# gmlwns2000/sharkshark-4k

Hardware: AMD Instinct MI355X
Metric: upscaled frames/sec at 720p->1440p x2 (whole job) (higher is better)
Workload: dtype f16; 1 GPU; RealESRGAN RRDBNet x2 (23 blocks) 720p->1440p fp16 [BASELINE configs[2]]; io=uint8 NHWC resident in HBM

## Files before the change

### include/ss4k_dev.h

```cpp
#ifndef SS4K_DEV_H
#define SS4K_DEV_H
#include "ss4k.h"
#ifdef __cplusplus
extern "C" {
#endif


int ss4k_bench_conv(ss4k_ctx* ctx, int dtype, int cin0, int cin1, int cout, int n, int h, int w, int flags,
                    int iters, double* avg_us, void* hip_stream);

int ss4k_dev_op_area_normalized(ss4k_ctx* ctx, const void* in, int in_half, float* out, int planes, int h, int w, int oh,
                                int ow, const float* st_hr, const float* st_lr, void* hip_stream);
int ss4k_dev_op_tail_fused(ss4k_ctx* ctx, void* hr, int hr_half, uint8_t* out_u8, const float* diff, int n, int c, int h,
                           int w, int dh, int dw, const float* st_hr, const float* st_lr, void* hip_stream);
int ss4k_dev_op_bicubic_u8(ss4k_ctx* ctx, const void* in, int in_half, uint8_t* out, int n, int c, int h, int w, int oh,
                           int ow, void* hip_stream);
int ss4k_dev_op_bicubic(ss4k_ctx* ctx, const float* in, float* out, int planes, int h, int w, int oh, int ow, int clamp01,
                        void* hip_stream);
int ss4k_dev_op_bilinear(ss4k_ctx* ctx, const float* in, float* out, int planes, int h, int w, int oh, int ow,
                         int subtract_from_out, int clamp01, void* hip_stream);
int ss4k_dev_gauss17_taps(float* taps17);
int ss4k_dev_op_gauss17_reflect(ss4k_ctx* ctx, const float* in, float* tmp, float* out, const float* taps17_dev, int planes,
                                int h, int w, void* hip_stream);
int ss4k_dev_op_depthwise_reflect(ss4k_ctx* ctx, const float* in, float* out, const float* taps_dev, int planes, int h,
                                  int w, int k, int clamp01, const float* blend_src, float blend_a, float blend_b,
                                  void* hip_stream);
int ss4k_dev_op_normalize(ss4k_ctx* ctx, float* x, const float* st_hr, const float* st_lr, int planes, int hw, void* hip_stream);
int ss4k_dev_op_sub(ss4k_ctx* ctx, const float* a, const float* b, float* out, size_t n, void* hip_stream);
int ss4k_dev_op_clamp01(ss4k_ctx* ctx, float* x, size_t n, void* hip_stream);
int ss4k_dev_op_plane_stats(ss4k_ctx* ctx, double* acc, const void* in, int in_half, float* stats, int planes, int hw,
                            void* hip_stream);
int ss4k_dev_op_plane_stats_u8nhwc(ss4k_ctx* ctx, double* acc, const uint8_t* in, float* stats, int n, int hw, void* hip_stream);
int ss4k_dev_op_plane_stats_partial(ss4k_ctx* ctx, double* acc, const void* in, int in_half, int planes, int hw,
                                    int acc_planes, int plane0, void* hip_stream);
int ss4k_dev_op_plane_stats_u8nhwc_partial(ss4k_ctx* ctx, double* acc, const uint8_t* in, int n, int hw, int acc_planes,
                                           int plane0, void* hip_stream);
int ss4k_dev_op_plane_stats_finish(ss4k_ctx* ctx, const double* acc, float* stats, int planes, int hw, void* hip_stream);
int ss4k_dev_op_plane_stats_finish2(ss4k_ctx* ctx, double* acc, float* stats_a, float* stats_b, int planes, int hw_a,
                                    int hw_b, int rezero, void* hip_stream);
int ss4k_dev_op_ps_nchw_addbase(ss4k_ctx* ctx, const void* src, int src_half, void* out, int out_half, const float* base,
                                int n, int h, int w, int r, int cq, double* stats_acc, void* hip_stream);
int ss4k_dev_op_pack_input(ss4k_ctx* ctx, const float* in, void* out, int out_half, int n, int c, int h, int w, int r,
                           int nplanes, void* hip_stream);
int ss4k_dev_op_temporal_shift(ss4k_ctx* ctx, const void* in, void* out, int nplanes, int frames, size_t frame_px,
                               int slots_per_record, int ch_per_plane, int fold, void* hip_stream);

int ss4k_dev_op_frvsr_maxpool2_planes(ss4k_ctx* ctx, const void* in, void* out, int half, int nplanes, int n, int h, int w, void* hip_stream);
int ss4k_dev_op_frvsr_bilinear2_planes(ss4k_ctx* ctx, const void* in, void* out, int half, int nplanes, int n, int h, int w, void* hip_stream);
int ss4k_dev_op_frvsr_flow_finish(ss4k_ctx* ctx, const float* raw, float* flow, int n, int h8, int w8, int h, int w, void* hip_stream);
int ss4k_dev_op_frvsr_warp_s2d_planes(ss4k_ctx* ctx, const float* lr_flow, const float* hr_prev, void* out, int half, int n, int h, int w,
                                      void* hip_stream);
int ss4k_dev_op_frvsr_warp_s2d_planes_items(ss4k_ctx* ctx, const float* lr_flow, const float* const* hr_prev, void* out, int half, int n,
                                            int h, int w, void* hip_stream);
int ss4k_dev_op_frvsr_ps4_conv_tail(ss4k_ctx* ctx, const void* in, int half, const float* wb, float* out, int n, int h, int w, void* hip_stream);
int ss4k_dev_op_frvsr_ps4_conv_tail_items(ss4k_ctx* ctx, const void* in, int half, const float* wb, float* const* out, int n, int h, int w,
                                          void* hip_stream);
int ss4k_dev_op_frvsr_planes_to_nchw(ss4k_ctx* ctx, const void* in, int half, float* out, int n, int channels, int h, int w, void* hip_stream);
int ss4k_dev_op_frvsr_clamp01_to(ss4k_ctx* ctx, const float* in, float* out, size_t n, void* hip_stream);
int ss4k_dev_op_frvsr_frames_in_items(ss4k_ctx* ctx, const uint8_t* const* in, float* const* lr_curr, int n, int h, int w, int lh, int lw,
                                      void* hip_stream);
int ss4k_dev_op_frvsr_pack_lr_items(ss4k_ctx* ctx, const float* const* lr_curr, const float* const* lr_prev, void* a, void* b, int half, int n,
                                    int h, int w, void* hip_stream);
int ss4k_dev_op_frvsr_frames_out_items(ss4k_ctx* ctx, const float* const* hr, uint8_t* const* out, int n, int H, int W, int oh, int ow,
                                       void* hip_stream);

int ss4k_dev_op_frvsrbi_bilinear_upsample4(ss4k_ctx* ctx, const float* in, float* out, int planes, int h, int w, void* hip_stream);
int ss4k_dev_op_frvsrbi_warp_s2d_planes(ss4k_ctx* ctx, const float* lr_flow, const float* hr_prev, void* out, int half, int n, int h, int w,
                                         void* hip_stream);
int ss4k_dev_op_frvsrbi_warp_s2d_planes_items(ss4k_ctx* ctx, const float* lr_flow, const float* const* hr_prev, void* out, int half, int n,
                                               int h, int w, void* hip_stream);
int ss4k_dev_op_frvsrbi_bilinear4_add(ss4k_ctx* ctx, const float* conv, const float* lr, float* out, int n, int h, int w, void* hip_stream);
int ss4k_dev_op_frvsrbi_bilinear4_add_items(ss4k_ctx* ctx, const float* conv, const float* const* lr, float* const* out, int n, int h, int w,
                                          void* hip_stream);

int ss4k_dev_frvsr_step_taps(ss4k_frvsr* m, const float* lr_curr, const float* lr_prev, const float* hr_prev, float* hr_out, float* flow_out,
                             float* s2d_out, int n, int h, int w, void* hip_stream);

int ss4k_dev_frvsr_tail_taps(ss4k_frvsr* m, const float* body_nchw, const float* lr_curr, float* up1_out, float* up2_out, float* hr_out, int n, int h,
                             int w, int max_workgroups, int group_items, void* hip_stream);
int ss4k_dev_frvsr_embed_convt(const float* wt_and_bias, int nf, float* out, size_t capacity_floats);
int ss4k_dev_frvsr_pack_convt(const float* wt, int dtype, void* out, size_t capacity_bytes);

int ss4k_dev_op_spin(ss4k_ctx* ctx, unsigned ticks, void* hip_stream);
int ss4k_dev_lane_handicap(ss4k_ctx* ctx, int lane, unsigned ticks);
int ss4k_dev_lane_counts(ss4k_ctx* ctx, int64_t* forks, int64_t* joins, int64_t* spins);
int ss4k_dev_lane_counts_reset(ss4k_ctx* ctx);
int ss4k_dev_lane_drop_join(ss4k_ctx* ctx, int k);

int ss4k_dev_glue_routes_reset(void);
int ss4k_dev_glue_routes_read(int index, char* name, size_t name_capacity, int64_t* launches);

int ss4k_dev_guard_enable(int on);
int ss4k_dev_guard_check(int* guarded, int* unguarded, int* damaged, char* text, size_t text_capacity);
int ss4k_dev_guard_poison(ss4k_ctx* ctx, ss4k_model* model, ss4k_upscaler* upscaler, int* buffers, size_t* bytes, size_t* bytes_256);
int ss4k_dev_guard_poison_frvsr(ss4k_frvsr* m, ss4k_frvsr_upscaler* up, int* buffers, size_t* bytes, size_t* bytes_256);
int ss4k_dev_guard_selftest(ss4k_ctx* ctx);

#ifdef __cplusplus
}
#endif
#endif
```

### sharkshark-4k_amd/_capi.py

```python
from __future__ import annotations

import ctypes as C
import os
from typing import Optional, Sequence, Tuple

import numpy as np
import torch

_HERE = os.path.dirname(os.path.abspath(__file__))
LIB_PATH = os.environ.get("SS4K_LIB") or os.path.join(_HERE, "libss4k_hip.so")

FSRCNN, RRDBNET, SRVGG, BSVD = 1, 2, 3, 4
F32, F16 = 0, 1

SYMBOLS = [
    "ss4k_abi_version", "ss4k_last_error", "ss4k_ctx_create", "ss4k_ctx_destroy", "ss4k_ctx_device",
    "ss4k_model_param_count", "ss4k_model_create", "ss4k_model_destroy", "ss4k_model_out_shape",
    "ss4k_model_in_channels", "ss4k_model_forward", "ss4k_model_check", "ss4k_upscaler_create", "ss4k_upscaler_destroy",
    "ss4k_upscaler_reset", "ss4k_upscaler_out_shape", "ss4k_upscaler_last_enqueue_ms", "ss4k_model_workspace_bytes", "ss4k_upscale_frames", "ss4k_upscaler_enable_taps",
    "ss4k_upscaler_read_tap", "ss4k_op_u8nhwc_to_f32nchw", "ss4k_op_area_resize", "ss4k_op_bicubic_resize",
    "ss4k_op_bilinear_resize", "ss4k_op_depthwise_reflect", "ss4k_op_plane_stats", "ss4k_op_f32nchw_to_u8nhwc",
    "ss4k_prof_enable", "ss4k_prof_reset", "ss4k_prof_read", "ss4k_prof_read_kind", "ss4k_prof_read_family", "ss4k_prof_read_section_ms",
    "ss4k_stream_pair_check", "ss4k_op_cv_area_shape", "ss4k_op_cv_area_resize_u8",
    "ss4k_frvsr_param_count", "ss4k_frvsr_create", "ss4k_frvsr_destroy", "ss4k_frvsr_step", "ss4k_frvsr_workspace_bytes",
    "ss4k_frvsr_prof_enable", "ss4k_frvsr_prof_read", "ss4k_frvsr_upscaler_create", "ss4k_frvsr_upscaler_destroy",
    "ss4k_frvsr_upscaler_reset", "ss4k_frvsr_upscaler_out_shape", "ss4k_frvsr_upscale_frames", "ss4k_frvsr_upscaler_enable_taps",
    "ss4k_frvsr_upscaler_read_tap", "ss4k_op_backward_warp", "ss4k_op_bicubic_upsample4",
    "ss4k_frvsr_upscaler_create_streams", "ss4k_frvsr_upscale_streams", "ss4k_frvsr_upscaler_reset_stream", "ss4k_frvsr_upscaler_state_bytes",
    "ss4k_frvsr_upscale_streams_at",
    "ss4k_frvsr_param_count_as", "ss4k_frvsr_create_as", "ss4k_frvsr_generator",
    "ss4k_frvsr_param_count_ex", "ss4k_frvsr_create_ex", "ss4k_frvsr_degradation",
]
DEV_SYMBOLS = [
    "ss4k_bench_conv",
    "ss4k_dev_op_area_normalized", "ss4k_dev_op_tail_fused", "ss4k_dev_op_bicubic_u8", "ss4k_dev_op_bicubic", "ss4k_dev_op_bilinear",
    "ss4k_dev_gauss17_taps", "ss4k_dev_op_gauss17_reflect", "ss4k_dev_op_depthwise_reflect", "ss4k_dev_op_normalize", "ss4k_dev_op_sub",
    "ss4k_dev_op_clamp01", "ss4k_dev_op_plane_stats", "ss4k_dev_op_plane_stats_u8nhwc", "ss4k_dev_op_plane_stats_partial",
    "ss4k_dev_op_plane_stats_u8nhwc_partial", "ss4k_dev_op_plane_stats_finish", "ss4k_dev_op_plane_stats_finish2",
    "ss4k_dev_op_ps_nchw_addbase", "ss4k_dev_op_pack_input", "ss4k_dev_op_temporal_shift",
    "ss4k_dev_glue_routes_reset", "ss4k_dev_glue_routes_read",
    "ss4k_dev_op_frvsr_maxpool2_planes", "ss4k_dev_op_frvsr_bilinear2_planes", "ss4k_dev_op_frvsr_flow_finish",
    "ss4k_dev_op_frvsr_warp_s2d_planes", "ss4k_dev_op_frvsr_warp_s2d_planes_items", "ss4k_dev_op_frvsr_ps4_conv_tail",
    "ss4k_dev_op_frvsr_ps4_conv_tail_items", "ss4k_dev_op_frvsr_planes_to_nchw", "ss4k_dev_op_frvsr_clamp01_to",
    "ss4k_dev_op_frvsr_frames_in_items", "ss4k_dev_op_frvsr_pack_lr_items", "ss4k_dev_op_frvsr_frames_out_items",
    "ss4k_dev_op_frvsrbi_bilinear_upsample4", "ss4k_dev_op_frvsrbi_warp_s2d_planes", "ss4k_dev_op_frvsrbi_warp_s2d_planes_items",
    "ss4k_dev_op_frvsrbi_bilinear4_add", "ss4k_dev_op_frvsrbi_bilinear4_add_items",
    "ss4k_dev_frvsr_step_taps",
    "ss4k_dev_frvsr_tail_taps", "ss4k_dev_frvsr_embed_convt", "ss4k_dev_frvsr_pack_convt",
    "ss4k_dev_guard_enable", "ss4k_dev_guard_check", "ss4k_dev_guard_poison", "ss4k_dev_guard_selftest", "ss4k_dev_guard_poison_frvsr",
    "ss4k_dev_op_spin", "ss4k_dev_lane_handicap", "ss4k_dev_lane_counts", "ss4k_dev_lane_counts_reset", "ss4k_dev_lane_drop_join",
]


class ModelDesc(C.Structure):
    _fields_ = [("kind", C.c_int32), ("dtype", C.c_int32), ("scale", C.c_int32), ("num_feat", C.c_int32),
                ("num_block", C.c_int32), ("num_grow_ch", C.c_int32), ("bsvd_chns", C.c_int32 * 3),
                ("bsvd_mid_ch", C.c_int32), ("bsvd_interm_ch", C.c_int32), ("bsvd_stream", C.c_int32),
                ("flags", C.c_int32), ("reserved", C.c_int32 * 3)]


MODEL_FS_EXACT, MODEL_ONE_CHAIN, MODEL_TWO_CHAINS, MODEL_TILE_ROWS_16, MODEL_TILE_ROWS_20 = 1, 2, 4, 16, 32
MODEL_NO_PAIR, MODEL_HR_F32, MODEL_NO_DENSE, MODEL_NO_WIDE, MODEL_NO_UPS_PRESUM, MODEL_NO_W16 = 256, 512, 1024, 4096, 8192, 32768
MODEL_FLAGS_ALL = 1 | 2 | 4 | 16 | 32 | 256 | 512 | 1024 | 4096 | 8192 | 32768


class UpscaleCfg(C.Structure):
    _fields_ = [("lr_h", C.c_int32), ("lr_w", C.c_int32), ("out_h", C.c_int32), ("out_w", C.c_int32),
                ("lr_hr_resize", C.c_int32), ("single_mode", C.c_int32), ("sr_is_realesrgan", C.c_int32),
                ("denoising", C.c_int32), ("reserved0", C.c_int32), ("denoise_rate", C.c_double),
                ("reserved", C.c_int32 * 6)]


class FrvsrDesc(C.Structure):
    _fields_ = [("dtype", C.c_int32), ("num_feat", C.c_int32), ("num_block", C.c_int32), ("flags", C.c_int32),
                ("reserved", C.c_int32 * 4)]


class Ss4kError(RuntimeError):
    pass


_lib = None
GPU_TOUCHED = False


def lib() -> C.CDLL:
    global _lib
    if _lib is None:
        _lib = load(LIB_PATH)
    return _lib


def load(path: str) -> C.CDLL:
    if not os.path.exists(path):
        raise Ss4kError(f"{path} is missing: build it with `python -c 'import __graft_entry__ as g; g.build()'`")
    L = C.CDLL(path)
    vp, i, sz = C.c_void_p, C.c_int, C.c_size_t
    L.ss4k_last_error.restype = C.c_char_p
    L.ss4k_ctx_create.argtypes = [i, C.POINTER(vp)]
    L.ss4k_ctx_destroy.argtypes = [vp]; L.ss4k_ctx_destroy.restype = None
    L.ss4k_ctx_device.argtypes = [vp]
    L.ss4k_model_param_count.argtypes = [C.POINTER(ModelDesc)]; L.ss4k_model_param_count.restype = sz
    L.ss4k_model_create.argtypes = [vp, C.POINTER(ModelDesc), vp, sz, C.POINTER(vp)]
    L.ss4k_model_destroy.argtypes = [vp]; L.ss4k_model_destroy.restype = None
    L.ss4k_model_out_shape.argtypes = [vp, i, i, i, C.POINTER(i), C.POINTER(i), C.POINTER(i)]
    L.ss4k_model_in_channels.argtypes = [vp]
    L.ss4k_model_forward.argtypes = [vp, vp, vp, i, i, i, vp]
    if hasattr(L, "ss4k_model_check"):
        L.ss4k_model_check.argtypes = [vp, i]
    L.ss4k_upscaler_create.argtypes = [vp, C.POINTER(UpscaleCfg), vp, vp, C.POINTER(vp)]
    L.ss4k_upscaler_destroy.argtypes = [vp]; L.ss4k_upscaler_destroy.restype = None
    L.ss4k_upscaler_reset.argtypes = [vp]
    L.ss4k_model_workspace_bytes.argtypes = [vp, i, i, i, C.POINTER(C.c_size_t)]
    L.ss4k_upscaler_last_enqueue_ms.argtypes = [vp, C.POINTER(C.c_double), C.POINTER(C.c_double)]
    L.ss4k_upscaler_out_shape.argtypes = [vp, i, i, i, C.POINTER(i), C.POINTER(i)]
    L.ss4k_upscale_frames.argtypes = [vp, vp, i, i, i, vp, sz, vp]
    L.ss4k_upscaler_enable_taps.argtypes = [vp, i]
    L.ss4k_upscaler_read_tap.argtypes = [vp, i, vp, sz, C.POINTER(i * 4), vp]
    L.ss4k_op_u8nhwc_to_f32nchw.argtypes = [vp, vp, vp, i, i, i, i, vp]
    for name in ("ss4k_op_area_resize", "ss4k_op_bicubic_resize", "ss4k_op_bilinear_resize"):
        getattr(L, name).argtypes = [vp, vp, vp, i, i, i, i, i, vp]
    L.ss4k_op_depthwise_reflect.argtypes = [vp, vp, vp, i, i, i, vp, i, vp]
    L.ss4k_op_plane_stats.argtypes = [vp, vp, vp, i, i, vp]
    L.ss4k_op_f32nchw_to_u8nhwc.argtypes = [vp, vp, vp, i, i, i, i, vp]
    if hasattr(L, "ss4k_bench_conv"):
        L.ss4k_bench_conv.argtypes = [vp, i, i, i, i, i, i, i, i, i, C.POINTER(C.c_double), vp]
    if hasattr(L, "ss4k_dev_glue_routes_read"):
        f = C.c_float
        L.ss4k_dev_op_area_normalized.argtypes = [vp, vp, i, vp, i, i, i, i, i, vp, vp, vp]
        L.ss4k_dev_op_tail_fused.argtypes = [vp, vp, i, vp, vp, i, i, i, i, i, i, vp, vp, vp]
        L.ss4k_dev_op_bicubic_u8.argtypes = [vp, vp, i, vp, i, i, i, i, i, i, vp]
        L.ss4k_dev_op_bicubic.argtypes = [vp, vp, vp, i, i, i, i, i, i, vp]
        L.ss4k_dev_op_bilinear.argtypes = [vp, vp, vp, i, i, i, i, i, i, i, vp]
        L.ss4k_dev_gauss17_taps.argtypes = [vp]
        L.ss4k_dev_op_gauss17_reflect.argtypes = [vp, vp, vp, vp, vp, i, i, i, vp]
        L.ss4k_dev_op_depthwise_reflect.argtypes = [vp, vp, vp, vp, i, i, i, i, i, vp, f, f, vp]
        L.ss4k_dev_op_normalize.argtypes = [vp, vp, vp, vp, i, i, vp]
        L.ss4k_dev_op_sub.argtypes = [vp, vp, vp, vp, sz, vp]
        L.ss4k_dev_op_clamp01.argtypes = [vp, vp, sz, vp]
        L.ss4k_dev_op_plane_stats.argtypes = [vp, vp, vp, i, vp, i, i, vp]
        L.ss4k_dev_op_plane_stats_u8nhwc.argtypes = [vp, vp, vp, vp, i, i, vp]
        L.ss4k_dev_op_plane_stats_partial.argtypes = [vp, vp, vp, i, i, i, i, i, vp]
        L.ss4k_dev_op_plane_stats_u8nhwc_partial.argtypes = [vp, vp, vp, i, i, i, i, vp]
        L.ss4k_dev_op_plane_stats_finish.argtypes = [vp, vp, vp, i, i, vp]
        L.ss4k_dev_op_plane_stats_finish2.argtypes = [vp, vp, vp, vp, i, i, i, i, vp]
        L.ss4k_dev_op_ps_nchw_addbase.argtypes = [vp, vp, i, vp, i, vp, i, i, i, i, i, vp, vp]
        L.ss4k_dev_op_pack_input.argtypes = [vp, vp, vp, i, i, i, i, i, i, i, vp]
        L.ss4k_dev_op_temporal_shift.argtypes = [vp, vp, vp, i, i, sz, i, i, i, vp]
        L.ss4k_dev_glue_routes_reset.argtypes = []
        L.ss4k_dev_op_frvsr_maxpool2_planes.argtypes = [vp, vp, vp, i, i, i, i, i, vp]
        L.ss4k_dev_op_frvsr_bilinear2_planes.argtypes = [vp, vp, vp, i, i, i, i, i, vp]
        L.ss4k_dev_op_frvsr_flow_finish.argtypes = [vp, vp, vp, i, i, i, i, i, vp]
        L.ss4k_dev_op_frvsr_warp_s2d_planes.argtypes = [vp, vp, vp, vp, i, i, i, i, vp]
        L.ss4k_dev_op_frvsr_warp_s2d_planes_items.argtypes = [vp, vp, vp, vp, i, i, i, i, vp]
        L.ss4k_dev_op_frvsr_ps4_conv_tail.argtypes = [vp, vp, i, vp, vp, i, i, i, vp]
        L.ss4k_dev_op_frvsr_ps4_conv_tail_items.argtypes = [vp, vp, i, vp, vp, i, i, i, vp]
        L.ss4k_dev_op_frvsr_planes_to_nchw.argtypes = [vp, vp, i, vp, i, i, i, i, vp]
        L.ss4k_dev_op_frvsr_clamp01_to.argtypes = [vp, vp, vp, sz, vp]
        L.ss4k_dev_op_frvsr_frames_in_items.argtypes = [vp, vp, vp, i, i, i, i, i, vp]
        L.ss4k_dev_op_frvsr_pack_lr_items.argtypes = [vp, vp, vp, vp, vp, i, i, i, i, vp]
        L.ss4k_dev_op_frvsr_frames_out_items.argtypes = [vp, vp, vp, i, i, i, i, i, vp]
        L.ss4k_dev_glue_routes_read.argtypes = [i, C.c_char_p, sz, C.POINTER(C.c_int64)]
    if hasattr(L, "ss4k_dev_op_frvsrbi_bilinear_upsample4"):
        L.ss4k_dev_op_frvsrbi_bilinear_upsample4.argtypes = [vp, vp, vp, i, i, i, vp]
        L.ss4k_dev_op_frvsrbi_warp_s2d_planes.argtypes = [vp, vp, vp, vp, i, i, i, i, vp]
        L.ss4k_dev_op_frvsrbi_warp_s2d_planes_items.argtypes = [vp, vp, vp, vp, i, i, i, i, vp]
        L.ss4k_dev_op_frvsrbi_bilinear4_add.argtypes = [vp, vp, vp, vp, i, i, i, vp]
        L.ss4k_dev_op_frvsrbi_bilinear4_add_items.argtypes = [vp, vp, vp, vp, i, i, i, vp]
    if hasattr(L, "ss4k_dev_frvsr_step_taps"):
        L.ss4k_dev_frvsr_step_taps.argtypes = [vp, vp, vp, vp, vp, vp, vp, i, i, i, vp]
    if hasattr(L, "ss4k_dev_guard_check"):
        L.ss4k_dev_guard_enable.argtypes = [i]
        L.ss4k_dev_guard_check.argtypes = [C.POINTER(i), C.POINTER(i), C.POINTER(i), C.c_char_p, sz]
        L.ss4k_dev_guard_poison.argtypes = [vp, vp, vp, C.POINTER(i), C.POINTER(sz), C.POINTER(sz)]
        L.ss4k_dev_guard_selftest.argtypes = [vp]
        if hasattr(L, "ss4k_dev_guard_poison_frvsr"):
            L.ss4k_dev_guard_poison_frvsr.argtypes = [vp, vp, C.POINTER(i), C.POINTER(sz), C.POINTER(sz)]
    if hasattr(L, "ss4k_dev_lane_counts"):
        i64p = C.POINTER(C.c_int64)
        L.ss4k_dev_op_spin.argtypes = [vp, C.c_uint, vp]
        L.ss4k_dev_lane_handicap.argtypes = [vp, i, C.c_uint]
        L.ss4k_dev_lane_counts.argtypes = [vp, i64p, i64p, i64p]
        L.ss4k_dev_lane_counts_reset.argtypes = [vp]
        L.ss4k_dev_lane_drop_join.argtypes = [vp, i]
    L.ss4k_prof_enable.argtypes = [vp, i]
    L.ss4k_prof_reset.argtypes = [vp]
    L.ss4k_prof_read.argtypes = [vp, C.POINTER(C.c_int64), C.POINTER(C.c_double), C.POINTER(C.c_double)]
    if hasattr(L, "ss4k_prof_read_kind"):
        L.ss4k_prof_read_kind.argtypes = [vp, i, C.POINTER(C.c_int64), C.POINTER(C.c_double), C.POINTER(C.c_double)]
    if hasattr(L, "ss4k_prof_read_family"):
        L.ss4k_prof_read_family.argtypes = [vp, i, C.c_char_p, sz, C.POINTER(C.c_int64), C.POINTER(C.c_double), C.POINTER(C.c_double)]
    L.ss4k_prof_read_section_ms.argtypes = [vp, C.POINTER(C.c_double)]
    L.ss4k_stream_pair_check.argtypes = [vp, vp, vp, C.POINTER(C.c_int)]
    L.ss4k_op_cv_area_shape.argtypes = [i, i, C.c_double, C.c_double, C.POINTER(C.c_int), C.POINTER(C.c_int)]
    L.ss4k_op_cv_area_resize_u8.argtypes = [vp, vp, vp, sz, i, i, i, i, C.c_double, C.c_double, vp]
    if hasattr(L, "ss4k_frvsr_create"):
        L.ss4k_frvsr_param_count.argtypes = [C.POINTER(FrvsrDesc)]; L.ss4k_frvsr_param_count.restype = sz
        L.ss4k_frvsr_create.argtypes = [vp, C.POINTER(FrvsrDesc), vp, sz, C.POINTER(vp)]
        L.ss4k_frvsr_destroy.argtypes = [vp]; L.ss4k_frvsr_destroy.restype = None
        L.ss4k_frvsr_step.argtypes = [vp, vp, vp, vp, vp, i, i, i, vp]
        L.ss4k_frvsr_workspace_bytes.argtypes = [vp, i, i, i, C.POINTER(C.c_size_t)]
        L.ss4k_frvsr_prof_enable.argtypes = [vp, i]
        L.ss4k_frvsr_prof_read.argtypes = [vp, i, C.POINTER(C.c_double)]
        L.ss4k_frvsr_upscaler_create.argtypes = [vp, vp, i, i, i, i, C.POINTER(vp)]
        L.ss4k_frvsr_upscaler_destroy.argtypes = [vp]; L.ss4k_frvsr_upscaler_destroy.restype = None
        L.ss4k_frvsr_upscaler_reset.argtypes = [vp]
        L.ss4k_frvsr_upscaler_out_shape.argtypes = [vp, C.POINTER(i), C.POINTER(i)]
        L.ss4k_frvsr_upscale_frames.argtypes = [vp, vp, i, i, i, vp, sz, vp]
        L.ss4k_frvsr_upscaler_enable_taps.argtypes = [vp, i]
        L.ss4k_frvsr_upscaler_read_tap.argtypes = [vp, i, vp, sz, C.POINTER(i * 4), vp]
        L.ss4k_op_backward_warp.argtypes = [vp, vp, vp, vp, i, i, i, i, vp]
        L.ss4k_op_bicubic_upsample4.argtypes = [vp, vp, vp, i, i, i, vp]
    if hasattr(L, "ss4k_frvsr_upscale_streams"):
        L.ss4k_frvsr_upscaler_create_streams.argtypes = [vp, vp, i, i, i, i, i, C.POINTER(vp)]
        L.ss4k_frvsr_upscale_streams.argtypes = [vp, C.POINTER(C.c_int32), i, vp, i, i, vp, sz, vp]
        L.ss4k_frvsr_upscaler_reset_stream.argtypes = [vp, i]
        L.ss4k_frvsr_upscaler_state_bytes.argtypes = [vp, C.POINTER(C.c_size_t)]
    if hasattr(L, "ss4k_frvsr_upscale_streams_at"):
        L.ss4k_frvsr_upscale_streams_at.argtypes = [vp, C.POINTER(C.c_int32), i, C.POINTER(vp), i, i, C.POINTER(vp), sz, vp]
    if hasattr(L, "ss4k_frvsr_create_as"):
        L.ss4k_frvsr_param_count_as.argtypes = [C.POINTER(FrvsrDesc), i]; L.ss4k_frvsr_param_count_as.restype = sz
        L.ss4k_frvsr_create_as.argtypes = [vp, C.POINTER(FrvsrDesc), i, i, vp, sz, C.POINTER(vp)]
        L.ss4k_frvsr_generator.argtypes = [vp]
    if hasattr(L, "ss4k_frvsr_create_ex"):
        L.ss4k_frvsr_param_count_ex.argtypes = [C.POINTER(FrvsrDesc), i, i]; L.ss4k_frvsr_param_count_ex.restype = sz
        L.ss4k_frvsr_create_ex.argtypes = [vp, C.POINTER(FrvsrDesc), i, i, i, vp, sz, C.POINTER(vp)]
        L.ss4k_frvsr_degradation.argtypes = [vp]
    if hasattr(L, "ss4k_dev_frvsr_tail_taps"):
        L.ss4k_dev_frvsr_tail_taps.argtypes = [vp, vp, vp, vp, vp, vp, i, i, i, i, i, vp]
        L.ss4k_dev_frvsr_embed_convt.argtypes = [vp, i, vp, sz]
        L.ss4k_dev_frvsr_pack_convt.argtypes = [vp, i, vp, sz]
    return L


def glue_routes(L: C.CDLL) -> dict:
    out, idx = {}, 0
    while True:
        name, n = C.create_string_buffer(256), C.c_int64()
        if L.ss4k_dev_glue_routes_read(idx, name, 256, C.byref(n)) != 0:
            return out
        out[name.value.decode()] = n.value
        idx += 1


def _guard_lib(L: Optional[C.CDLL]) -> C.CDLL:
    L = L or lib()
    if not hasattr(L, "ss4k_dev_guard_check"):
        raise Ss4kError("guard mode lives in libss4k_hip_dev.so: run with SS4K_LIB=<package>/libss4k_hip_dev.so")
    return L


def _guard_rc(L: C.CDLL, rc: int) -> None:
    if rc != 0:
        raise Ss4kError(f"libss4k_hip_dev error {rc}: {L.ss4k_last_error().decode()}")


def guard_enable(on: bool = True, L: Optional[C.CDLL] = None) -> None:
    L = _guard_lib(L)
    _guard_rc(L, L.ss4k_dev_guard_enable(int(on)))


def guard_check(L: Optional[C.CDLL] = None) -> Tuple[int, int, int, str]:
    L = _guard_lib(L)
    g, u, d, text = C.c_int(), C.c_int(), C.c_int(), C.create_string_buffer(512)
    _guard_rc(L, L.ss4k_dev_guard_check(C.byref(g), C.byref(u), C.byref(d), text, 512))
    return g.value, u.value, d.value, text.value.decode()


def guard_poison(ctx=None, model=None, upscaler=None, L: Optional[C.CDLL] = None) -> Tuple[int, int, int]:
    L = _guard_lib(L)
    h = [getattr(o, "_h", o) for o in (ctx, model, upscaler)]
    n, b, b256 = C.c_int(), C.c_size_t(), C.c_size_t()
    _guard_rc(L, L.ss4k_dev_guard_poison(*h, C.byref(n), C.byref(b), C.byref(b256)))
    return n.value, int(b.value), int(b256.value)


def guard_poison_frvsr(model=None, upscaler=None, L: Optional[C.CDLL] = None) -> Tuple[int, int, int]:
    L = _guard_lib(L)
    h = [getattr(o, "_h", o) for o in (model, upscaler)]
    n, b, b256 = C.c_int(), C.c_size_t(), C.c_size_t()
    _guard_rc(L, L.ss4k_dev_guard_poison_frvsr(*h, C.byref(n), C.byref(b), C.byref(b256)))
    return n.value, int(b.value), int(b256.value)


def guard_selftest(ctx, L: Optional[C.CDLL] = None) -> None:
    L = _guard_lib(L)
    _guard_rc(L, L.ss4k_dev_guard_selftest(getattr(ctx, "_h", ctx)))


def _check(rc: int) -> None:
    if rc != 0:
        raise Ss4kError(f"libss4k_hip error {rc}: {lib().ss4k_last_error().decode()}")


def _stream() -> int:
    return int(torch.cuda.current_stream().cuda_stream)


def _dev_index(device) -> int:
    d = torch.device(device if not isinstance(device, int) else f"cuda:{device}")
    return d.index if d.index is not None else torch.cuda.current_device()


class Context:

    def __init__(self, device=0):
        self.device_index = _dev_index(device)
        self.device = torch.device("cuda", self.device_index)
        h = C.c_void_p()
        global GPU_TOUCHED
        rc = lib().ss4k_ctx_create(self.device_index, C.byref(h))
        GPU_TOUCHED = GPU_TOUCHED or rc == 0 or torch.cuda.device_count() > 0
        _check(rc)
        self._h = h

    def close(self):
        if getattr(self, "_h", None):
            lib().ss4k_ctx_destroy(self._h)
            self._h = None

    def __del__(self):
        try:
            self.close()
        except Exception:
            pass

    def prof_enable(self, on: bool):
        _check(lib().ss4k_prof_enable(self._h, int(on)))

    def prof_reset(self):
        _check(lib().ss4k_prof_reset(self._h))

    def prof_read(self) -> Tuple[int, float, float]:
        n, ms, fl = C.c_int64(), C.c_double(), C.c_double()
        _check(lib().ss4k_prof_read(self._h, C.byref(n), C.byref(ms), C.byref(fl)))
        return n.value, ms.value, fl.value

# ... 436 lines not shown
```

### sharkshark-4k_amd/csrc/conv_w16n.hip

```cpp
#include "common.h"
#include "conv_tile.h"
#include <type_traits>

namespace ss4k {
namespace w16n {

typedef float f32x4 __attribute__((ext_vector_type(4)));

constexpr int NW = 4, MB = 4, TH = NW * MB;
constexpr int XH = TH + 2, XW = TW + 2;
constexpr int REC = 32;
constexpr int ROWX = XW * REC;
constexpr int XT_SLOTS = XH * XW * 2;
constexpr int XT_BYTES = XT_SLOTS * 16;
constexpr int XT_DMA = (XT_SLOTS + 63) / 64;
constexpr int DMA_PER_WAVE = (XT_DMA + NW - 1) / NW;
constexpr int WP = 3 * 1024, NWS = 3;
constexpr int NDMA = DMA_PER_WAVE + 1;
constexpr int W_OFF = 2 * XT_BYTES, B_OFF = W_OFF + NWS * WP;
constexpr size_t LDS_BYTES = B_OFF + 16 * 4;
static_assert(3 * LDS_BYTES <= 160 * 1024, "three workgroups per CU");

__device__ __forceinline__ f32x4 mma16(const uint4& w, const uint4& x, f32x4 acc) {
  return __builtin_amdgcn_mfma_f32_16x16x32_f16(__builtin_bit_cast(f16x8, w), __builtin_bit_cast(f16x8, x), acc, 0, 0, 0);
}

__global__ __launch_bounds__(64 * NW, 3) void conv3x3_w16n_kernel(const ConvArgs a) {
  extern __shared__ __attribute__((aligned(16))) char smem[];
  const uint32_t lds0 = (uint32_t)(size_t)(__attribute__((address_space(3))) char*)smem;
  const int tid = threadIdx.x, lane = tid & 63;
  const int wave = __builtin_amdgcn_readfirstlane(tid >> 6);
  const int n16 = lane & 15, kg = lane >> 4;
  const int K = a.nchunks0 + a.nchunks1, NP = K >> 1;
  const int ntiles = a.N * a.tiles_y * a.tiles_x;
  const char* wbase = reinterpret_cast<const char*>(a.w16);

  const bool banded = (gridDim.x % 8 == 0) && ntiles >= (int)gridDim.x;
  const int tpx = (ntiles + 7) / 8;
  auto tile_of = [&](int k) __attribute__((always_inline)) -> int {
    if (!banded) {
      const int t = blockIdx.x + k * gridDim.x;
      return t < ntiles ? (a.reverse ? ntiles - 1 - t : t) : -1;
    }
    const int base = (blockIdx.x & 7) * tpx, len = min(tpx, ntiles - base);
    const int j = (blockIdx.x >> 3) + k * (gridDim.x >> 3);
    return j < len ? base + (a.reverse ? len - 1 - j : j) : -1;
  };
  int rdA[2], rdX[2];
#pragma unroll
  for (int hn = 0; hn < 2; ++hn) {
    rdA[hn] = (((wave * MB) * XW + 16 * hn + n16 + (kg >> 1)) * 2 + (kg & 1)) * 16;
    rdX[hn] = (((wave * MB) * XW + 16 * hn + n16 + 2) * 2 + (kg & 1)) * 16 + (kg >> 1) * XT_BYTES;
  }
  auto setup_tile = [&](int tile, int& n, int& y0, int& x0) __attribute__((always_inline)) {
    const int tx = tile % a.tiles_x, tyn = tile / a.tiles_x;
    const int ty = tyn % a.tiles_y;
    n = a.n0 + tyn / a.tiles_y; y0 = ty * TH; x0 = tx * TW;
  };
  auto tile_src = [&](int k, int n, int y0, int x0) __attribute__((always_inline)) -> uint32_t {
    int ln = lane;
    asm volatile("" : "+v"(ln));
    const int s = k * 64 + ln;
    const int p = s >> 1, gq = s & 1;
    const int row = p / XW, x = p - row * XW;
    const int iy = y0 - 1 + row, ix = x0 - 1 + x;
    const bool ok = s < XT_SLOTS && iy >= 0 && iy < a.H && ix >= 0 && ix < a.W;
    return ok ? ((uint32_t)(n * a.H + iy) * (uint32_t)a.W + (uint32_t)ix) * REC + (uint32_t)(gq * 16) : OOB;
  };
  auto plane_of = [&](int c) __attribute__((always_inline)) {
    return (c < a.nchunks0) ? a.in0 + (size_t)(a.in0_plane0 + c) * a.in0_plane_bytes
                            : a.in1 + (size_t)(a.in1_plane0 + c - a.nchunks0) * a.in1_plane_bytes;
  };
  const char* pf_plane = nullptr; const char* pf_w = nullptr; int pf_buf = 0, pf_slot = 0, pf_n = 0, pf_y0 = 0, pf_x0 = 0; bool pf_tile = false, pf_wt = false;
  auto dma_op = [&](int idx) __attribute__((always_inline)) {
    if (idx < DMA_PER_WAVE) {
      const int k = wave + NW * idx;
      if (pf_tile && k < XT_DMA) {
        const uint32_t so = tile_src(k, pf_n, pf_y0, pf_x0);
        const char* src = so != OOB ? pf_plane + so : a.zero_page + (lane & 3) * 16;
        const uint32_t dst = __builtin_amdgcn_readfirstlane(lds0 + pf_buf * XT_BYTES + k * 1024);
        if (k * 64 + lane < XT_SLOTS) dma16(src, dst);
      }
    } else if (idx < NDMA) {
      int l16 = lane * 16;
      asm volatile("" : "+v"(l16));
      if (pf_wt && wave < 3) dma16(pf_w + wave * 1024 + l16, __builtin_amdgcn_readfirstlane(lds0 + W_OFF + pf_slot * WP + wave * 1024));
    }
  };
  auto slot_inc = [](int s) { return s == NWS - 1 ? 0 : s + 1; };

  float* bias_lds = reinterpret_cast<float*>(smem + B_OFF);
  if (tid < 16) bias_lds[tid] = tid < a.cout_pad ? a.bias[tid] : 0.f;

  int kt = 0;
  int tile = tile_of(0);
  if (tile < 0) return;
  int n, y0, x0;
  setup_tile(tile, n, y0, x0);
  pf_n = n; pf_y0 = y0; pf_x0 = x0;
  int ws = 0;
  pf_tile = true; pf_plane = plane_of(0); pf_buf = 0; pf_wt = true; pf_w = wbase; pf_slot = 0;
#pragma unroll
  for (int i = 0; i < NDMA; ++i) dma_op(i);
  pf_tile = false; pf_w = wbase + WP; pf_slot = 1;
  dma_op(DMA_PER_WAVE);
  dma_wait();
  __syncthreads();
  const int lane16 = lane * 16;
  uint4 wf[3];
#pragma unroll
  for (int dy = 0; dy < 3; ++dy) wf[dy] = *reinterpret_cast<const uint4*>(smem + W_OFF + lane16 + dy * 1024);

  while (true) {
    f32x4 acc[MB][2];
    f32x4 bias4;
    {
      const float4* bp = reinterpret_cast<const float4*>(smem + B_OFF + kg * 16);
      int o = 0;
      asm volatile("" : "+v"(o));
      const float4 b0 = bp[o];
      bias4 = f32x4{b0.x, b0.y, b0.z, b0.w};
    }
    const int cur_n = n, cur_y0 = y0, cur_x0 = x0;
    const int next_tile = tile_of(kt + 1);

    auto period = [&](const int q, auto FIRSTP) __attribute__((always_inline)) {
      const bool last_q = q + 1 == NP;
      auto phase = [&](auto PH, auto FIRST) __attribute__((always_inline)) {
        constexpr int ph = decltype(PH)::value;
        constexpr bool first = decltype(FIRST)::value;
        const int lp2 = 3 * q + ph + 2;
        if (lp2 < 3 * NP) { pf_wt = true; pf_w = wbase + (size_t)lp2 * WP; }
        else if (next_tile >= 0) { pf_wt = true; pf_w = wbase + (size_t)(lp2 - 3 * NP) * WP; }
        else pf_wt = false;
        pf_slot = ws == 0 ? NWS - 1 : ws - 1;
        if constexpr (ph == 0) { pf_tile = true; pf_plane = plane_of(2 * q + 1); pf_buf = 1; }
        else if constexpr (ph == 1) { pf_tile = false; }
        else {
          pf_buf = 0;
          if (!last_q) { pf_tile = true; pf_plane = plane_of(2 * q + 2); }
          else if (next_tile >= 0) { setup_tile(next_tile, n, y0, x0); pf_n = n; pf_y0 = y0; pf_x0 = x0; pf_tile = true; pf_plane = plane_of(0); }
          else pf_tile = false;
        }
        const bool more = !(last_q && ph == 2) || next_tile >= 0;
        const char* tb = smem + (ph == 2 ? XT_BYTES : 0);
        const int* rd = ph == 1 ? rdX : rdA;
        const char* wbn = smem + W_OFF + slot_inc(ws) * WP + lane16;
        uint4 bf[3][2];
        auto bf_load = [&](int t, int hn) __attribute__((always_inline)) { return *reinterpret_cast<const uint4*>(tb + rd[hn] + t * ROWX); };
#pragma unroll
        for (int t = 0; t < 3; ++t) { bf[t][0] = bf_load(t, 0); bf[t][1] = bf_load(t, 1); }
        int m = 0;
        __builtin_amdgcn_sched_barrier(0);
#pragma unroll
        for (int ir = 0; ir < MB + 2; ++ir) {
#pragma unroll
          for (int dy = 0; dy < 3; ++dy) {
            const int r = ir - dy;
            if (r >= 0 && r < MB) {
#pragma unroll
              for (int hn = 0; hn < 2; ++hn) {
                acc[r][hn] = mma16(wf[dy], bf[ir % 3][hn], (first && dy == 0) ? bias4 : acc[r][hn]);
                if ((m & 3) == 3) {
                  __builtin_amdgcn_sched_barrier(0);
                  dma_op(m >> 2);
                  __builtin_amdgcn_sched_barrier(0);
                }
                ++m;
              }
            }
          }
          __builtin_amdgcn_sched_barrier(0);
          if (ir + 3 < MB + 2) { bf[ir % 3][0] = bf_load(ir + 3, 0); bf[ir % 3][1] = bf_load(ir + 3, 1); }
          if (more && ir >= MB - 1) wf[ir - (MB - 1)] = *reinterpret_cast<const uint4*>(wbn + (ir - (MB - 1)) * 1024);
          __builtin_amdgcn_sched_barrier(0);
        }
        if (more) { dma_wait(); __syncthreads(); }
        ws = slot_inc(ws);
      };
      phase(std::integral_constant<int, 0>{}, FIRSTP);
      phase(std::integral_constant<int, 1>{}, std::false_type{});
      phase(std::integral_constant<int, 2>{}, std::false_type{});
    };
    period(0, std::true_type{});
#pragma unroll 1
    for (int q = 1; q < NP; ++q) period(q, std::false_type{});

    if (kg == 0) {
      float* o = reinterpret_cast<float*>(a.out);
      const size_t plane = (size_t)a.H * a.W;
#pragma unroll
      for (int r = 0; r < MB; ++r) {
        const int y = cur_y0 + wave * MB + r;
#pragma unroll
        for (int hn = 0; hn < 2; ++hn) {
          const int x = cur_x0 + 16 * hn + n16;
          if (y < a.H && x < a.W) {
#pragma unroll
            for (int i = 0; i < 4; ++i)
              if (i < a.cout_real) o[((size_t)cur_n * a.cout_real + i) * plane + (size_t)y * a.W + x] = acc[r][hn][i];
          }
        }
      }
    }
    if (next_tile < 0) break;
    tile = next_tile; ++kt;
  }
}

}

bool conv3x3_w16n_eligible(const ConvArgs& a, int dtype) {
  return dtype == SS4K_F16 && a.w16 && a.epi == EPI_NCHW_F32 && a.cout_real <= 4 && a.act == ACT_NONE && !a.res1 && !a.res2 && !a.bsvd_resid &&
         a.alpha == 1.f && !a.dbg && !a.ups2 && (a.nchunks0 + a.nchunks1) % 2 == 0 && conv_plane_span_f16(a) < 4294967296.0;
}

void launch_conv3x3_w16n(ss4k_ctx* ctx, const ConvArgs& a0, hipStream_t st) {
  using namespace w16n;
  ConvArgs a = a0;
  a.tiles_x = (a.W + TW - 1) / TW; a.tiles_y = (a.H + TH - 1) / TH;
  a.zero_page = ctx->zero_page();
  const int ntiles = a.N * a.tiles_y * a.tiles_x;
  const int gx = std::min(ntiles, std::max(1, (int)(ctx->num_cu * 3 * (a.grid_share > 0.f ? a.grid_share : 1.f))));
  const void* fn = reinterpret_cast<const void*>(&conv3x3_w16n_kernel);
  if (ctx->lds_attr_set.insert(fn).second)
    SS4K_HIP(hipFuncSetAttribute(fn, hipFuncAttributeMaxDynamicSharedMemorySize, (int)LDS_BYTES));
  ctx->prof_family = "w16n::conv3x3_w16n_kernel (one 16-cout block, 16x16x32 MFMA, NCHW fp32 hand-off: a final 64 -> 3 layer)";
  hipLaunchKernelGGL(conv3x3_w16n_kernel, dim3(gx), dim3(64 * NW), LDS_BYTES, st, a);
  SS4K_HIP(hipGetLastError());
}

}
```

Measured before the change: 126.2 frames/s.

## Keep all conv weights resident in LDS and triple-buffer input planes across tiles

The final 64->3 conv kernel now loads the full weight set into LDS once and uses three rotating input-plane slots. The next plane, including the first planes of the next tile, is prefetched with counted vmcnt waits, so there is no drain between tiles. The cost is more LDS per workgroup, which drops occupancy from three to two workgroups per CU. The old kernel is kept as a dev-only drain variant behind an environment variable, and a dev entry point is added for benchmarking.

Result: no change. 126.4 frames/s, median of 6 (+0.2%).

```diff
diff --git a/include/ss4k_dev.h b/include/ss4k_dev.h
--- a/include/ss4k_dev.h
+++ b/include/ss4k_dev.h
@@ -8,6 +8,9 @@
 
 int ss4k_bench_conv(ss4k_ctx* ctx, int dtype, int cin0, int cin1, int cout, int n, int h, int w, int flags,
                     int iters, double* avg_us, void* hip_stream);
+
+int ss4k_dev_conv_w16n(ss4k_ctx* ctx, const void* planes_f16, const float* w_oihw, const float* bias, float* out_nchw, int k_chunks, int cout,
+                       int n, int h, int w, int reverse, int max_workgroups, void* hip_stream);
 
 int ss4k_dev_op_area_normalized(ss4k_ctx* ctx, const void* in, int in_half, float* out, int planes, int h, int w, int oh,
                                 int ow, const float* st_hr, const float* st_lr, void* hip_stream);
diff --git a/sharkshark-4k_amd/_capi.py b/sharkshark-4k_amd/_capi.py
--- a/sharkshark-4k_amd/_capi.py
+++ b/sharkshark-4k_amd/_capi.py
@@ -33,6 +33,7 @@
 ]
 DEV_SYMBOLS = [
     "ss4k_bench_conv",
+    "ss4k_dev_conv_w16n",
     "ss4k_dev_op_area_normalized", "ss4k_dev_op_tail_fused", "ss4k_dev_op_bicubic_u8", "ss4k_dev_op_bicubic", "ss4k_dev_op_bilinear",
     "ss4k_dev_gauss17_taps", "ss4k_dev_op_gauss17_reflect", "ss4k_dev_op_depthwise_reflect", "ss4k_dev_op_normalize", "ss4k_dev_op_sub",
     "ss4k_dev_op_clamp01", "ss4k_dev_op_plane_stats", "ss4k_dev_op_plane_stats_u8nhwc", "ss4k_dev_op_plane_stats_partial",
diff --git a/sharkshark-4k_amd/csrc/conv_w16n.hip b/sharkshark-4k_amd/csrc/conv_w16n.hip
--- a/sharkshark-4k_amd/csrc/conv_w16n.hip
+++ b/sharkshark-4k_amd/csrc/conv_w16n.hip
@@ -1,5 +1,8 @@
 #include "common.h"
 #include "conv_tile.h"
+#ifdef SS4K_DEV
+#include "api_guard.h"
+#endif
 #include <type_traits>
 
 namespace ss4k {
@@ -15,17 +18,221 @@
 constexpr int XT_BYTES = XT_SLOTS * 16;
 constexpr int XT_DMA = (XT_SLOTS + 63) / 64;
 constexpr int DMA_PER_WAVE = (XT_DMA + NW - 1) / NW;
-constexpr int WP = 3 * 1024, NWS = 3;
+constexpr int WP = 3 * 1024;
+constexpr int NSLOT = 3;
+constexpr int W_OFF = NSLOT * XT_BYTES;
+constexpr int LDS_CU = 160 * 1024;
+constexpr size_t lds_bytes(int K) { return (size_t)W_OFF + (size_t)(K / 2) * 3 * WP + 16 * 4; }
+static_assert(XT_DMA == NW * DMA_PER_WAVE, "every wave issues DMA_PER_WAVE LDS-DMAs per plane: the counted waits rely on it");
+static_assert(2 * lds_bytes(4) <= LDS_CU, "two workgroups per CU for a 64-channel input");
+
+__device__ __forceinline__ f32x4 mma16(const uint4& w, const uint4& x, f32x4 acc) {
+  return __builtin_amdgcn_mfma_f32_16x16x32_f16(__builtin_bit_cast(f16x8, w), __builtin_bit_cast(f16x8, x), acc, 0, 0, 0);
+}
+template <int N> __device__ __forceinline__ void dma_wait_but() { asm volatile("s_waitcnt vmcnt(%0)" ::"n"(N) : "memory"); }
+
+__global__ __launch_bounds__(64 * NW, 2) void conv3x3_w16n_kernel(const ConvArgs a) {
+  extern __shared__ __attribute__((aligned(16))) char smem[];
+  const uint32_t lds0 = (uint32_t)(size_t)(__attribute__((address_space(3))) char*)smem;
+  const int tid = threadIdx.x, lane = tid & 63;
+  const int wave = __builtin_amdgcn_readfirstlane(tid >> 6);
+  const int n16 = lane & 15, kg = lane >> 4;
+  const int K = a.nchunks0 + a.nchunks1, NP = K >> 1, NPH = 3 * NP;
+  const int b_off = W_OFF + NPH * WP;
+  const int ntiles = a.N * a.tiles_y * a.tiles_x;
+  const char* wbase = reinterpret_cast<const char*>(a.w16);
+
+  const bool banded = (gridDim.x % 8 == 0) && ntiles >= (int)gridDim.x;
+  const int tpx = (ntiles + 7) / 8;
+  auto tile_of = [&](int k) __attribute__((always_inline)) -> int {
+    if (!banded) {
+      const int t = blockIdx.x + k * gridDim.x;
+      return t < ntiles ? (a.reverse ? ntiles - 1 - t : t) : -1;
+    }
+    const int base = (blockIdx.x & 7) * tpx, len = min(tpx, ntiles - base);
+    const int j = (blockIdx.x >> 3) + k * (gridDim.x >> 3);
+    return j < len ? base + (a.reverse ? len - 1 - j : j) : -1;
+  };
+  int rdA[2], rdX[2];
+#pragma unroll
+  for (int hn = 0; hn < 2; ++hn) {
+    rdA[hn] = (((wave * MB) * XW + 16 * hn + n16 + (kg >> 1)) * 2 + (kg & 1)) * 16;
+    rdX[hn] = (((wave * MB) * XW + 16 * hn + n16 + 2) * 2 + (kg & 1)) * 16;
+  }
+  auto setup_tile = [&](int tile, int& n, int& y0, int& x0) __attribute__((always_inline)) {
+    const int tx = tile % a.tiles_x, tyn = tile / a.tiles_x;
+    const int ty = tyn % a.tiles_y;
+    n = a.n0 + tyn / a.tiles_y; y0 = ty * TH; x0 = tx * TW;
+  };
+  int prow[DMA_PER_WAVE], pcol[DMA_PER_WAVE];
+  uint32_t poff[DMA_PER_WAVE];
+#pragma unroll
+  for (int i = 0; i < DMA_PER_WAVE; ++i) {
+    const int s = (wave + NW * i) * 64 + lane;
+    const int p = s >> 1, gq = s & 1;
+    const int row = p / XW;
+    prow[i] = s < XT_SLOTS ? row : (1 << 28);
+    pcol[i] = p - row * XW;
+    poff[i] = ((uint32_t)row * (uint32_t)a.W + (uint32_t)pcol[i]) * REC + (uint32_t)(gq * 16);
+  }
+  auto plane_of = [&](int c) __attribute__((always_inline)) {
+    return (c < a.nchunks0) ? a.in0 + (size_t)(a.in0_plane0 + c) * a.in0_plane_bytes
+                            : a.in1 + (size_t)(a.in1_plane0 + c - a.nchunks0) * a.in1_plane_bytes;
+  };
+  auto request_piece = [&](int i, const char* plane, int slot, int n, int y0, int x0) __attribute__((always_inline)) {
+    const uint32_t origin = ((uint32_t)(n * a.H + y0 - 1) * (uint32_t)a.W + (uint32_t)(x0 - 1)) * REC;
+    const bool ok = (uint32_t)(prow[i] + y0 - 1) < (uint32_t)a.H && (uint32_t)(pcol[i] + x0 - 1) < (uint32_t)a.W;
+    const char* src = ok ? plane + (uint32_t)(origin + poff[i]) : a.zero_page + (lane & 3) * 16;
+    const int k = wave + NW * i;
+    const uint32_t dst = __builtin_amdgcn_readfirstlane(lds0 + slot * XT_BYTES + k * 1024);
+    if (k * 64 + lane < XT_SLOTS) dma16(src, dst);
+  };
+  auto request = [&](const char* plane, int slot, int n, int y0, int x0) __attribute__((always_inline)) {
+#pragma unroll
+    for (int i = 0; i < DMA_PER_WAVE; ++i) request_piece(i, plane, slot, n, y0, x0);
+  };
+  auto slot_inc = [](int s) { return s == NSLOT - 1 ? 0 : s + 1; };
+
+  float* bias_lds = reinterpret_cast<float*>(smem + b_off);
+  if (tid < 16) bias_lds[tid] = tid < a.cout_pad ? a.bias[tid] : 0.f;
+
+  int kt = 0;
+  int tile = tile_of(0);
+  if (tile < 0) return;
+  int n, y0, x0;
+  setup_tile(tile, n, y0, x0);
+  int next_tile = tile_of(1);
+  int nn = 0, ny0 = 0, nx0 = 0;
+  if (next_tile >= 0) setup_tile(next_tile, nn, ny0, nx0);
+  const int lane16 = lane * 16;
+  for (int i = wave; i < 3 * NPH; i += NW) {
+    int l16 = lane16;
+    asm volatile("" : "+v"(l16));
+    dma16(wbase + (size_t)i * 1024 + l16, __builtin_amdgcn_readfirstlane(lds0 + W_OFF + i * 1024));
+  }
+  request(plane_of(0), 0, n, y0, x0);
+  request(plane_of(1), 1, n, y0, x0);
+  dma_wait_but<DMA_PER_WAVE>();
+  lds_barrier();
+  int sa = 0;
+  uint4 wf[3];
+#pragma unroll
+  for (int dy = 0; dy < 3; ++dy) wf[dy] = *reinterpret_cast<const uint4*>(smem + W_OFF + lane16 + dy * 1024);
+
+  while (true) {
+    f32x4 acc[MB][2];
+    f32x4 bias4;
+    {
+      const float4* bp = reinterpret_cast<const float4*>(smem + b_off + kg * 16);
+      int o = 0;
+      asm volatile("" : "+v"(o));
+      const float4 b0 = bp[o];
+      bias4 = f32x4{b0.x, b0.y, b0.z, b0.w};
+    }
+
+    auto period = [&](const int q, auto FIRSTP) __attribute__((always_inline)) {
+      const bool last_q = q + 1 == NP;
+      const int sb = slot_inc(sa), sc = slot_inc(sb);
+      auto phase = [&](auto PH, auto FIRST) __attribute__((always_inline)) {
+        constexpr int ph = decltype(PH)::value;
+        constexpr bool first = decltype(FIRST)::value;
+        bool requested = false;
+        const char* rq_plane = nullptr; int rq_slot = 0, rq_n = n, rq_y0 = y0, rq_x0 = x0;
+        if constexpr (ph != 1) {
+          const int c = 2 * q + (ph == 0 ? 2 : 3);
+          rq_slot = ph == 0 ? sc : sa;
+          if (c < K) { rq_plane = plane_of(c); requested = true; }
+          else if (next_tile >= 0) { rq_plane = plane_of(c - K); rq_n = nn; rq_y0 = ny0; rq_x0 = nx0; requested = true; }
+        }
+        const bool more = !(last_q && ph == 2) || next_tile >= 0;
+        const int np = 3 * q + ph + 1;
+        const char* wbn = smem + W_OFF + (np == NPH ? 0 : np) * WP + lane16;
+        const int so = (ph == 0 ? sa : ph == 2 ? sb : (kg >> 1) ? sb : sa) * XT_BYTES;
+        const int* rd = ph == 1 ? rdX : rdA;
+        const char* tb[2] = {smem + so + rd[0], smem + so + rd[1]};
+        uint4 bf[3][2];
+        auto bf_load = [&](int t, int hn) __attribute__((always_inline)) { return *reinterpret_cast<const uint4*>(tb[hn] + t * ROWX); };
+        __builtin_amdgcn_sched_barrier(0);
+#pragma unroll
+        for (int t = 0; t < 3; ++t) { bf[t][0] = bf_load(t, 0); bf[t][1] = bf_load(t, 1); }
+        int m = 0;
+        __builtin_amdgcn_sched_barrier(0);
+#pragma unroll
+        for (int ir = 0; ir < MB + 2; ++ir) {
+#pragma unroll
+          for (int dy = 0; dy < 3; ++dy) {
+            const int r = ir - dy;
+            if (r >= 0 && r < MB) {
+#pragma unroll
+              for (int hn = 0; hn < 2; ++hn) {
+                acc[r][hn] = mma16(wf[dy], bf[ir % 3][hn], (first && dy == 0) ? bias4 : acc[r][hn]);
+                if constexpr (ph != 1) {
+                  if ((m & 3) == 1 && (m >> 2) < DMA_PER_WAVE) {
+                    __builtin_amdgcn_sched_barrier(0);
+                    if (requested) request_piece(m >> 2, rq_plane, rq_slot, rq_n, rq_y0, rq_x0);
+                    __builtin_amdgcn_sched_barrier(0);
+                  }
+                }
+                ++m;
+              }
+            }
+          }
+          __builtin_amdgcn_sched_barrier(0);
+          if (ir + 3 < MB + 2) { bf[ir % 3][0] = bf_load(ir + 3, 0); bf[ir % 3][1] = bf_load(ir + 3, 1); }
+          if (more && ir >= MB - 1) wf[ir - (MB - 1)] = *reinterpret_cast<const uint4*>(wbn + (ir - (MB - 1)) * 1024);
+          __builtin_amdgcn_sched_barrier(0);
+        }
+        if (more) {
+          if constexpr (ph != 1) {
+            if (requested) dma_wait_but<DMA_PER_WAVE>(); else dma_wait_but<0>();
+          }
+          lds_barrier();
+        }
+      };
+      phase(std::integral_constant<int, 0>{}, FIRSTP);
+      phase(std::integral_constant<int, 1>{}, std::false_type{});
+      phase(std::integral_constant<int, 2>{}, std::false_type{});
+      sa = sc;
+    };
+    period(0, std::true_type{});
+#pragma unroll 1
+    for (int q = 1; q < NP; ++q) period(q, std::false_type{});
+
+    if (kg == 0) {
+      float* o = reinterpret_cast<float*>(a.out);
+      const size_t plane = (size_t)a.H * a.W;
+#pragma unroll
+      for (int r = 0; r < MB; ++r) {
+        const int y = y0 + wave * MB + r;
+#pragma unroll
+        for (int hn = 0; hn < 2; ++hn) {
+          const int x = x0 + 16 * hn + n16;
+          if (y < a.H && x < a.W) {
+#pragma unroll
+            for (int i = 0; i < 4; ++i)
+              if (i < a.cout_real) o[((size_t)n * a.cout_real + i) * plane + (size_t)y * a.W + x] = acc[r][hn][i];
+          }
+        }
+      }
+    }
+    if (next_tile < 0) break;
+    tile = next_tile; ++kt;
+    n = nn; y0 = ny0; x0 = nx0;
+    next_tile = tile_of(kt + 1);
+    if (next_tile >= 0) setup_tile(next_tile, nn, ny0, nx0);
+  }
+}
+
+#ifdef SS4K_DEV
+namespace drain {
+
+constexpr int NWS = 3;
 constexpr int NDMA = DMA_PER_WAVE + 1;
 constexpr int W_OFF = 2 * XT_BYTES, B_OFF = W_OFF + NWS * WP;
 constexpr size_t LDS_BYTES = B_OFF + 16 * 4;
 static_assert(3 * LDS_BYTES <= 160 * 1024, "three workgroups per CU");
 
-__device__ __forceinline__ f32x4 mma16(const uint4& w, const uint4& x, f32x4 acc) {
-  return __builtin_amdgcn_mfma_f32_16x16x32_f16(__builtin_bit_cast(f16x8, w), __builtin_bit_cast(f16x8, x), acc, 0, 0, 0);
-}
-
-__global__ __launch_bounds__(64 * NW, 3) void conv3x3_w16n_kernel(const ConvArgs a) {
+__global__ __launch_bounds__(64 * NW, 3) void conv3x3_w16n_drain_kernel(const ConvArgs a) {
   extern __shared__ __attribute__((aligned(16))) char smem[];
   const uint32_t lds0 = (uint32_t)(size_t)(__attribute__((address_space(3))) char*)smem;
   const int tid = threadIdx.x, lane = tid & 63;
@@ -209,10 +416,14 @@
 }
 
 }
+#endif
+
+}
 
 bool conv3x3_w16n_eligible(const ConvArgs& a, int dtype) {
   return dtype == SS4K_F16 && a.w16 && a.epi == EPI_NCHW_F32 && a.cout_real <= 4 && a.act == ACT_NONE && !a.res1 && !a.res2 && !a.bsvd_resid &&
-         a.alpha == 1.f && !a.dbg && !a.ups2 && (a.nchunks0 + a.nchunks1) % 2 == 0 && conv_plane_span_f16(a) < 4294967296.0;
+         a.alpha == 1.f && !a.dbg && !a.ups2 && (a.nchunks0 + a.nchunks1) % 2 == 0 && w16n::lds_bytes(a.nchunks0 + a.nchunks1) <= (size_t)w16n::LDS_CU &&
+         conv_plane_span_f16(a) < 4294967296.0;
 }
 
 void launch_conv3x3_w16n(ss4k_ctx* ctx, const ConvArgs& a0, hipStream_t st) {
@@ -221,13 +432,66 @@
   a.tiles_x = (a.W + TW - 1) / TW; a.tiles_y = (a.H + TH - 1) / TH;
   a.zero_page = ctx->zero_page();
   const int ntiles = a.N * a.tiles_y * a.tiles_x;
-  const int gx = std::min(ntiles, std::max(1, (int)(ctx->num_cu * 3 * (a.grid_share > 0.f ? a.grid_share : 1.f))));
+  const float share = a.grid_share > 0.f ? a.grid_share : 1.f;
+  ctx->prof_family = "w16n::conv3x3_w16n_kernel (one 16-cout block, 16x16x32 MFMA, NCHW fp32 hand-off: a final 64 -> 3 layer)";
+#ifdef SS4K_DEV
+  static const bool drain_build = std::getenv("SS4K_W16N_DRAIN") && std::getenv("SS4K_W16N_DRAIN")[0] == '1';
+  if (drain_build) {
+    const int gx = std::min(ntiles, std::max(1, (int)(ctx->num_cu * 3 * share)));
+    const void* fn = reinterpret_cast<const void*>(&drain::conv3x3_w16n_drain_kernel);
+    if (ctx->lds_attr_set.insert(fn).second)
+      SS4K_HIP(hipFuncSetAttribute(fn, hipFuncAttributeMaxDynamicSharedMemorySize, (int)drain::LDS_BYTES));
+    hipLaunchKernelGGL(drain::conv3x3_w16n_drain_kernel, dim3(gx), dim3(64 * NW), drain::LDS_BYTES, st, a);
+    SS4K_HIP(hipGetLastError());
+    return;
+  }
+#endif
+  const size_t lds = lds_bytes(a.nchunks0 + a.nchunks1);
+  const int per_cu = std::max(1, std::min(2, (int)(LDS_CU / lds)));
+  const int gx = std::min(ntiles, std::max(1, (int)(ctx->num_cu * per_cu * share)));
   const void* fn = reinterpret_cast<const void*>(&conv3x3_w16n_kernel);
   if (ctx->lds_attr_set.insert(fn).second)
-    SS4K_HIP(hipFuncSetAttribute(fn, hipFuncAttributeMaxDynamicSharedMemorySize, (int)LDS_BYTES));
-  ctx->prof_family = "w16n::conv3x3_w16n_kernel (one 16-cout block, 16x16x32 MFMA, NCHW fp32 hand-off: a final 64 -> 3 layer)";
-  hipLaunchKernelGGL(conv3x3_w16n_kernel, dim3(gx), dim3(64 * NW), LDS_BYTES, st, a);
+    SS4K_HIP(hipFuncSetAttribute(fn, hipFuncAttributeMaxDynamicSharedMemorySize, LDS_CU));
+  hipLaunchKernelGGL(conv3x3_w16n_kernel, dim3(gx), dim3(64 * NW), lds, st, a);
   SS4K_HIP(hipGetLastError());
 }
 
 }
+
+#ifdef SS4K_DEV
+extern "C" int ss4k_dev_conv_w16n(ss4k_ctx* ctx, const void* planes_f16, const float* w_oihw, const float* bias, float* out_nchw, int k_chunks, int cout,
+                                  int n, int h, int w, int reverse, int max_workgroups, void* hip_stream) {
+  using namespace ss4k;
+  return guard([&] {
+    SS4K_REQUIRE(ctx && planes_f16 && w_oihw && bias && out_nchw, "NULL argument");
+    SS4K_REQUIRE(k_chunks >= 2 && k_chunks % 2 == 0 && cout >= 1 && cout <= 16 && n >= 1 && h >= 1 && w >= 1 && max_workgroups >= 0, "argument out of range");
+    hipStream_t st = (hipStream_t)hip_stream;
+    PackSpec s{};
+    s.dtype = SS4K_F16; s.cout_real = cout; s.cin_total = 16 * k_chunks; s.nchunks0 = k_chunks; s.nchunks1 = 0; s.ps2 = 0;
+    s.cin_map.resize((size_t)16 * k_chunks);
+    for (size_t i = 0; i < s.cin_map.size(); ++i) s.cin_map[i] = (int)i;
+    const std::vector<uint8_t> blob = pack_conv3x3_w16n(s, w_oihw);
+    float bias16[16] = {};
+    std::memcpy(bias16, bias, sizeof(float) * cout);
+    DevBuf& wb = ctx->buf("dev_conv_w16n_w", blob.size() + sizeof bias16);
+    SS4K_HIP(hipStreamSynchronize(st));
+    SS4K_HIP(hipMemcpy(wb.ptr, blob.data(), blob.size(), hipMemcpyHostToDevice));
+    SS4K_HIP(hipMemcpy(wb.as<char>() + blob.size(), bias16, sizeof bias16, hipMemcpyHostToDevice));
+    ConvArgs a{};
+    a.in0 = static_cast<const char*>(planes_f16); a.in0_plane_bytes = (size_t)n * h * w * 32; a.in0_plane0 = 0; a.nchunks0 = k_chunks;
+    a.N = n; a.H = h; a.W = w; a.n0 = 0; a.job_n = n;
+    a.w16 = wb.ptr; a.bias = reinterpret_cast<const float*>(wb.as<char>() + blob.size());
+    a.act = ACT_NONE; a.alpha = 1.f; a.gamma = 1.f;
+    a.epi = EPI_NCHW_F32; a.out = reinterpret_cast<char*>(out_nchw);
+    a.cout_real = std::min(cout, 4); a.cout_pad = 16;
+    a.reverse = reverse ? 1 : 0;
+    SS4K_REQUIRE(conv3x3_w16n_eligible(a, SS4K_F16), "not a layer of conv_w16n.hip");
+    if (max_workgroups > 0) {
+      const bool drain_build = std::getenv("SS4K_W16N_DRAIN") && std::getenv("SS4K_W16N_DRAIN")[0] == '1';
+      const int per_cu = drain_build ? 3 : std::max(1, std::min(2, (int)(w16n::LDS_CU / w16n::lds_bytes(k_chunks))));
+      a.grid_share = (max_workgroups + 0.5f) / (float)(ctx->num_cu * per_cu);
+    }
+    launch_conv3x3_w16n(ctx, a, st);
+  });
+}
+#endif
```
